# Jason9339/Wavelet-Noise-in-ray-tracing

Measured on AMD Instinct MI355X. Metric: Mnoise-samples/sec (3D wavelet, octave=4), higher is better.
Workload: dtype f32; 1 GPU; 512^3 dense 3D WNoise grid, tile=128, octave=4 (configs[1]); tile=128, seed=12345, octave=4, device=AMD Radeon Graphics (gfx950:sramecc+:xnack-)

## Files before the change

wavelet-noise-in-ray-tracing_amd/csrc/wn_wavelet_exact.hip:

```cpp
#include "wn_internal.hpp"

#include <algorithm>
#include <cmath>

namespace {

using wn::GridArgs;

typedef float v4f __attribute__((ext_vector_type(4)));

constexpr int kEX = 256, kEY = 8, kEZ = 8;
constexpr int kWaves = 4;
constexpr int kMaxBoxFloats = 12 * 1024;

struct ExactArgs {
    const float *coef;
    float *out;
    int n, nmask;
    GridArgs g;
    int nbx, nby, nbz;
    int vec4_ok;
    int box_cap;
};

__global__ __launch_bounds__(64 * kWaves) void grid3d_exact_lds_kernel(const ExactArgs a)
{
    extern __shared__ float box[];
    __shared__ int s_geo[8];
    const GridArgs &g = a.g;
    const float den = (float)g.den;
    const int tid = threadIdx.x, lane = tid & 63;
    const int wave = __builtin_amdgcn_readfirstlane(tid >> 6);
    const int bx = blockIdx.x, by = blockIdx.y, bz = blockIdx.z;
    const int x_first = bx * kEX, y_first = by * kEY, z_first = bz * kEZ;
    auto coord = [&](int i) { return wn::lattice_coord(i, den, g.base_range, g.octave_scale, g.post_scale); };
    auto zcoord = [&](int zi) { return g.z_const_mode ? g.z_const : coord(g.z0 + zi); };

    if (tid < 3) {
        const int lo_i = tid == 0 ? x_first : (tid == 1 ? y_first : z_first);
        const int n_i = tid == 0 ? g.nx : (tid == 1 ? g.ny : g.nz);
        const int hi_i = min(lo_i + (tid == 0 ? kEX : (tid == 1 ? kEY : kEZ)), n_i) - 1;
        const float c_lo = tid == 2 ? zcoord(lo_i) : coord(lo_i), c_hi = tid == 2 ? zcoord(hi_i) : coord(hi_i);
        int m_lo, m_hi;
        float w0, w1, w2;
        wn::bspline(c_lo, m_lo, w0, w1, w2);
        wn::bspline(c_hi, m_hi, w0, w1, w2);
        s_geo[tid] = min(m_lo, m_hi) - 1;
        s_geo[3 + tid] = abs(m_hi - m_lo) + 3;
    }
    __syncthreads();
    const int ix0 = s_geo[0], jy0 = s_geo[1], kz0 = s_geo[2];
    const int ex = s_geo[3], ey = s_geo[4], ez = s_geo[5];
    if ((long long)ex * ey * ez > a.box_cap) return;

    const int nrows = ey * ez;
    for (int r = wave; r < nrows; r += kWaves) {
        const int k = r / ey, j = r - k * ey;
        const float *row = a.coef + ((size_t)wn::dmod(kz0 + k, a.n, a.nmask) * a.n + wn::dmod(jy0 + j, a.n, a.nmask)) * a.n;
        for (int i = lane; i < ex; i += 64) box[r * ex + i] = row[wn::dmod(ix0 + i, a.n, a.nmask)];
    }

    const int x0 = x_first + lane * 4;
    int cx[4];
    float wx[4][3];
#pragma unroll
    for (int q = 0; q < 4; ++q) {
        int m;
        wn::bspline(coord(min(x0 + q, g.nx - 1)), m, wx[q][0], wx[q][1], wx[q][2]);
        cx[q] = m - 1 - ix0;
    }
    __syncthreads();

    const int rows_y = min(kEY, g.ny - y_first), rows_z = min(kEZ, g.nz - z_first);
    for (int r = wave; r < rows_y * rows_z; r += kWaves) {
        const int yi = r % rows_y, zi = r / rows_y;
        int my, mz;
        float wy[3], wz[3];
        wn::bspline(coord(y_first + yi), my, wy[0], wy[1], wy[2]);
        wn::bspline(zcoord(z_first + zi), mz, wz[0], wz[1], wz[2]);
        const int jrow = my - 1 - jy0, krow = mz - 1 - kz0;
        float res[4] = {0.0f, 0.0f, 0.0f, 0.0f};
#pragma unroll
        for (int fz = 0; fz < 3; ++fz)
#pragma unroll
            for (int fy = 0; fy < 3; ++fy) {
                const float *rowp = box + ((krow + fz) * ey + (jrow + fy)) * ex;
#pragma unroll
                for (int q = 0; q < 4; ++q) {
                    const float *c = rowp + cx[q];
#pragma unroll
                    for (int fx = 0; fx < 3; ++fx) {
                        const float weight = wx[q][fx] * wy[fy] * wz[fz];
                        res[q] += weight * c[fx];
                    }
                }
            }
        float *dst = a.out + ((size_t)(z_first + zi) * g.ny + (y_first + yi)) * g.nx + x0;
        if (a.vec4_ok && x0 + 3 < g.nx) {
            *reinterpret_cast<v4f *>(dst) = v4f{res[0] * g.out_scale, res[1] * g.out_scale, res[2] * g.out_scale, res[3] * g.out_scale};
        } else {
#pragma unroll
            for (int q = 0; q < 4; ++q)
                if (x0 + q < g.nx) dst[q] = res[q] * g.out_scale;
        }
    }
}

}

namespace wn {

int exact_lds_try(const wn_tile *tile, const GridArgs &g, float *out_dev, hipStream_t stream)
{
    if (tile->n == 0 || g.nx <= 0 || g.ny <= 0 || g.nz <= 0) return kDeclined;
    if (g.nx < 64) return kDeclined;
    LatticeStep ls;
    if (!lattice_step(g, g.octave_scale, true, true, 1.0, &ls)) return kDeclined;
    const long long ez = g.z_const_mode ? 3 : ls.extent(kEZ);
    const long long box_floats = ls.extent(kEX) * ls.extent(kEY) * ez;
    if (box_floats > kMaxBoxFloats) return kDeclined;
    ExactArgs a{};
    a.coef = tile->dev;
    a.out = out_dev;
    a.n = tile->n;
    a.nmask = pow2_mask(tile->n);
    a.g = g;
    a.nbx = (g.nx + kEX - 1) / kEX;
    a.nby = (g.ny + kEY - 1) / kEY;
    a.nbz = (g.nz + kEZ - 1) / kEZ;
    if (a.nby > 65535 || a.nbz > 65535) return kDeclined;
    a.vec4_ok = vec4_ok(out_dev, g.nx);
    a.box_cap = (int)box_floats;
    const size_t lds = (size_t)box_floats * sizeof(float);
    hipLaunchKernelGGL(grid3d_exact_lds_kernel, dim3(a.nbx, a.nby, a.nbz), dim3(64 * kWaves), lds, stream, a);
    WN_LAUNCH_CHECK("grid3d_exact_lds_kernel");
    return WN_OK;
}

}
```

Baseline: 1.384 million Msamples/s.

## Pair adjacent z rows to share LDS loads and use packed float2 FMAs

Each wave now owns a y row and walks z, precomputing the 36 x*y weights once per y row instead of recomputing weights per output row. When two consecutive z samples fall into the same or adjacent lattice cells, both outputs are computed together with packed v2f FMAs that reuse the same LDS coefficient reads. This is meant to cut LDS traffic and weight-multiply work. In exchange it adds branching on the z step and higher register pressure from the held weight vectors, which asm volatile barriers keep pinned in registers.

```diff
diff --git a/wavelet-noise-in-ray-tracing_amd/csrc/wn_wavelet_exact.hip b/wavelet-noise-in-ray-tracing_amd/csrc/wn_wavelet_exact.hip
--- a/wavelet-noise-in-ray-tracing_amd/csrc/wn_wavelet_exact.hip
+++ b/wavelet-noise-in-ray-tracing_amd/csrc/wn_wavelet_exact.hip
@@ -7,6 +7,7 @@
 
 using wn::GridArgs;
 
+typedef float v2f __attribute__((ext_vector_type(2)));
 typedef float v4f __attribute__((ext_vector_type(4)));
 
 constexpr int kEX = 256, kEY = 8, kEZ = 8;
@@ -72,29 +73,8 @@
     __syncthreads();
 
     const int rows_y = min(kEY, g.ny - y_first), rows_z = min(kEZ, g.nz - z_first);
-    for (int r = wave; r < rows_y * rows_z; r += kWaves) {
-        const int yi = r % rows_y, zi = r / rows_y;
-        int my, mz;
-        float wy[3], wz[3];
-        wn::bspline(coord(y_first + yi), my, wy[0], wy[1], wy[2]);
-        wn::bspline(zcoord(z_first + zi), mz, wz[0], wz[1], wz[2]);
-        const int jrow = my - 1 - jy0, krow = mz - 1 - kz0;
-        float res[4] = {0.0f, 0.0f, 0.0f, 0.0f};
-#pragma unroll
-        for (int fz = 0; fz < 3; ++fz)
-#pragma unroll
-            for (int fy = 0; fy < 3; ++fy) {
-                const float *rowp = box + ((krow + fz) * ey + (jrow + fy)) * ex;
-#pragma unroll
-                for (int q = 0; q < 4; ++q) {
-                    const float *c = rowp + cx[q];
-#pragma unroll
-                    for (int fx = 0; fx < 3; ++fx) {
-                        const float weight = wx[q][fx] * wy[fy] * wz[fz];
-                        res[q] += weight * c[fx];
-                    }
-                }
-            }
+    auto store_row = [&](int yi, int zi, float r0, float r1, float r2, float r3) {
+        const float res[4] = {r0, r1, r2, r3};
         float *dst = a.out + ((size_t)(z_first + zi) * g.ny + (y_first + yi)) * g.nx + x0;
         if (a.vec4_ok && x0 + 3 < g.nx) {
             *reinterpret_cast<v4f *>(dst) = v4f{res[0] * g.out_scale, res[1] * g.out_scale, res[2] * g.out_scale, res[3] * g.out_scale};
@@ -102,6 +82,114 @@
 #pragma unroll
             for (int q = 0; q < 4; ++q)
                 if (x0 + q < g.nx) dst[q] = res[q] * g.out_scale;
+        }
+    };
+
+    const int plane = ey * ex;
+#pragma unroll 1
+    for (int yi = wave; yi < rows_y; yi += kWaves) {
+        int my;
+        float wy[3];
+        wn::bspline(coord(y_first + yi), my, wy[0], wy[1], wy[2]);
+        const float *ybase = box + (my - 1 - jy0) * ex;
+        v2f wxy[18];
+#pragma unroll
+        for (int t = 0; t < 36; ++t) {
+            const float w = wx[t / 3 % 4][t % 3] * wy[t / 12];
+            if (t & 1) wxy[t >> 1].y = w;
+            else wxy[t >> 1].x = w;
+        }
+        auto w1 = [&](int fy, int q, int fx) {
+            const int t = (fy * 4 + q) * 3 + fx;
+            return (t & 1) ? wxy[t >> 1].y : wxy[t >> 1].x;
+        };
+        auto w2 = [&](int fy, int q, int fx) {
+            const int t = (fy * 4 + q) * 3 + fx;
+            return (t & 1) ? __builtin_shufflevector(wxy[t >> 1], wxy[t >> 1], 1, 1) : __builtin_shufflevector(wxy[t >> 1], wxy[t >> 1], 0, 0);
+        };
+
+#pragma unroll 1
+        for (int zi = 0; zi < rows_z;) {
+#pragma unroll
+            for (int t = 0; t < 18; ++t) asm volatile("" : "+v"(wxy[t]));
+            int mzA, s = -1;
+            float wzA[3], wzB[3] = {0.0f, 0.0f, 0.0f};
+            wn::bspline(zcoord(z_first + zi), mzA, wzA[0], wzA[1], wzA[2]);
+            if (!g.z_const_mode && zi + 1 < rows_z) {
+                int mzB;
+                wn::bspline(zcoord(z_first + zi + 1), mzB, wzB[0], wzB[1], wzB[2]);
+                s = mzB - mzA;
+            }
+            const float *pa = ybase + (mzA - 1 - kz0) * plane;
+            if (s == 0) {
+                v2f res[4] = {v2f{0.0f, 0.0f}, v2f{0.0f, 0.0f}, v2f{0.0f, 0.0f}, v2f{0.0f, 0.0f}};
+#pragma unroll
+                for (int fz = 0; fz < 3; ++fz) {
+                    const v2f wz2 = v2f{wzA[fz], wzB[fz]};
+#pragma unroll
+                    for (int fy = 0; fy < 3; ++fy) {
+                        const float *rowp = pa + fz * plane + fy * ex;
+#pragma unroll
+                        for (int q = 0; q < 4; ++q) {
+                            const float *c = rowp + cx[q];
+#pragma unroll
+                            for (int fx = 0; fx < 3; ++fx) {
+                                const v2f weight = w2(fy, q, fx) * wz2;
+                                res[q] += weight * v2f{c[fx], c[fx]};
+                            }
+                        }
+                    }
+                }
+                store_row(yi, zi, res[0].x, res[1].x, res[2].x, res[3].x);
+                store_row(yi, zi + 1, res[0].y, res[1].y, res[2].y, res[3].y);
+                zi += 2;
+            } else if (s == 1) {
+                v2f res[4] = {v2f{0.0f, 0.0f}, v2f{0.0f, 0.0f}, v2f{0.0f, 0.0f}, v2f{0.0f, 0.0f}};
+#pragma unroll
+                for (int r = 0; r < 4; ++r) {
+#pragma unroll
+                    for (int fy = 0; fy < 3; ++fy) {
+                        const float *rowp = pa + r * plane + fy * ex;
+#pragma unroll
+                        for (int q = 0; q < 4; ++q) {
+                            const float *c = rowp + cx[q];
+#pragma unroll
+                            for (int fx = 0; fx < 3; ++fx) {
+                                if (r == 0) {
+                                    res[q].x += w1(fy, q, fx) * wzA[0] * c[fx];
+                                } else if (r == 3) {
+                                    res[q].y += w1(fy, q, fx) * wzB[2] * c[fx];
+                                } else {
+                                    const v2f weight = w2(fy, q, fx) * v2f{wzA[r], wzB[r - 1]};
+                                    res[q] += weight * v2f{c[fx], c[fx]};
+                                }
+                            }
+                        }
+                    }
+                }
+                store_row(yi, zi, res[0].x, res[1].x, res[2].x, res[3].x);
+                store_row(yi, zi + 1, res[0].y, res[1].y, res[2].y, res[3].y);
+                zi += 2;
+            } else {
+                float res[4] = {0.0f, 0.0f, 0.0f, 0.0f};
+#pragma unroll
+                for (int fz = 0; fz < 3; ++fz)
+#pragma unroll
+                    for (int fy = 0; fy < 3; ++fy) {
+                        const float *rowp = pa + fz * plane + fy * ex;
+#pragma unroll
+                        for (int q = 0; q < 4; ++q) {
+                            const float *c = rowp + cx[q];
+#pragma unroll
+                            for (int fx = 0; fx < 3; ++fx) {
+                                const float weight = w1(fy, q, fx) * wzA[fz];
+                                res[q] += weight * c[fx];
+                            }
+                        }
+                    }
+                store_row(yi, zi, res[0], res[1], res[2], res[3]);
+                zi += 1;
+            }
         }
     }
 }
```

Measured after the change: 1.363 million Msamples/s. 0.985x the previous value.
